# uber-research/UPSNet

Hardware: NVIDIA H100
Metric: panoptic images/sec at 1024x2048 (higher is better)
Workload: dtype bf16x3

## Files before the change

### upsnet_b200/build.py

```python
import os
import shutil
import subprocess
import sys

HERE = os.path.dirname(os.path.abspath(__file__))
CSRC = os.path.join(HERE, "csrc")
LIB = os.path.join(HERE, "libupsnet_b200.so")
SOURCES = ["roi_align.cu", "nms.cu", "panoptic.cu", "igemm_simt.cu", "igemm_tc.cu", "igemm_tma.cu", "dcn_win.cu", "detection.cu", "pool.cu", "post.cu", "impost.cu", "pq.cu", "sseg.cu", "cocoeval.cu", "combined.cu", "rpn_target.cu", "proposal_target.cu", "panoptic_loss.cu", "train_loss.cu", "labels.cu", "backward.cu", "conv_backward.cu", "sgd.cu", "capi.cu"]
NVCC_FLAGS = ["-gencode", "arch=compute_90a,code=sm_90a", "-O3", "-lineinfo", "-std=c++17",
              "-Xcompiler", "-fPIC", "--expt-relaxed-constexpr"]


def nvcc():
    for home in (os.environ.get("CUDA_HOME"), os.environ.get("CUDA_PATH")):
        if home and os.path.exists(os.path.join(home, "bin", "nvcc")):
            return os.path.join(home, "bin", "nvcc")
    return shutil.which("nvcc") or "/usr/local/cuda/bin/nvcc"


def _stale():
    if not os.path.exists(LIB):
        return True
    t = os.path.getmtime(LIB)
    deps = [os.path.join(CSRC, f) for f in os.listdir(CSRC)]
    deps.append(os.path.join(HERE, "..", "include", "upsnet_b200.h"))
    return any(os.path.getmtime(d) > t for d in deps)


def build(force=False, verbose=False):
    if not force and not _stale():
        return LIB
    objs = []
    procs = []
    os.makedirs(os.path.join(HERE, "build"), exist_ok=True)
    for src in SOURCES:
        obj = os.path.join(HERE, "build", src.replace(".cu", ".o"))
        cmd = [nvcc()] + NVCC_FLAGS + (["-Xptxas", "-v"] if verbose else []) + \
              ["-c", os.path.join(CSRC, src), "-o", obj]
        procs.append((src, subprocess.Popen(cmd, stdout=subprocess.PIPE, stderr=subprocess.STDOUT, text=True)))
        objs.append(obj)
    failed = False
    for src, pr in procs:
        out, _ = pr.communicate()
        if pr.returncode != 0 or verbose:
            sys.stderr.write("== %s ==\n%s\n" % (src, out))
        failed |= pr.returncode != 0
    if failed:
        raise RuntimeError("nvcc failed")
    subprocess.check_call([nvcc()] + NVCC_FLAGS[:2] + ["-shared", "-o", LIB] + objs + ["-lcudart"])
    return LIB


if __name__ == "__main__":
    print(build(force="--force" in sys.argv, verbose="-v" in sys.argv))
```

### upsnet_b200/csrc/igemm_tc.cu

```cuda
#include <cuda_bf16.h>
#include <cstdio>

#include "common.cuh"
#include "tc_ptx.cuh"
#include "tc_params.cuh"

namespace ups {

constexpr int TC_BM = 128;
constexpr int TC_BK = 64;
constexpr int TC_GROUP = 256;
constexpr int TC_GROUPS = 2;
constexpr int TC_PRODUCERS = TC_GROUP * TC_GROUPS;
constexpr int TC_CONSUMERS = 128;
constexpr int TC_EPI_PITCH = 36;
constexpr int TC_THREADS = TC_CONSUMERS + TC_PRODUCERS;
constexpr int TC_MAX_STAGES = 6;



struct TcSmem {
  uint32_t bars;
  uint32_t rowbase;
  uint32_t epi;
// ... 527 lines not shown
            size_t ridx = oidx;
            if (p.res_up2) {
              const int ho = pp / p.Wo, wo = pp - ho * p.Wo;
              ridx = (((size_t)n_img * (p.Ho >> 1) + (ho >> 1)) * (p.Wo >> 1) + (wo >> 1)) * p.Cout + co0;
            }
            const bool full = (co0 + 15 < p.Cout) && ((p.Cout & 7) == 0) && vec_ptrs_ok;
            if (p.y_bf16) {
              __nv_bfloat16* yo = reinterpret_cast<__nv_bfloat16*>(p.y) + oidx;
              const __nv_bfloat16* ro = p.residual ? reinterpret_cast<const __nv_bfloat16*>(p.residual) + ridx : nullptr;
              if (full) {
                if (ro) {
                  const uint4 r0 = __ldg(reinterpret_cast<const uint4*>(ro)), r1 = __ldg(reinterpret_cast<const uint4*>(ro) + 1);
                  const uint32_t rw[8] = {r0.x, r0.y, r0.z, r0.w, r1.x, r1.y, r1.z, r1.w};
#pragma unroll
                  for (int q = 0; q < 8; ++q) {
                    o16[2 * q] += bf16x2_x(rw[q]);
                    o16[2 * q + 1] += bf16x2_y(rw[q]);
                  }
                }
                if (p.relu) {
#pragma unroll
                  for (int e = 0; e < 16; ++e) o16[e] = fmaxf(o16[e], 0.f);
                }
                reinterpret_cast<uint4*>(yo)[0] = pack_bf16x8(o16);
                reinterpret_cast<uint4*>(yo)[1] = pack_bf16x8(o16 + 8);
              } else {
#pragma unroll
                for (int e = 0; e < 16; ++e) {
                  if (co0 + e >= p.Cout) break;
                  float o = o16[e];
                  if (ro) o += __bfloat162float(ro[e]);
                  if (p.relu) o = fmaxf(o, 0.f);
                  yo[e] = __float2bfloat16_rn(o);
                }
              }
            } else {
              float* yo = reinterpret_cast<float*>(p.y) + oidx;
              const float* ro = p.residual ? reinterpret_cast<const float*>(p.residual) + ridx : nullptr;
              if (full) {
#pragma unroll
                for (int g4 = 0; g4 < 4; ++g4) {
                  float4 o = make_float4(o16[g4 * 4], o16[g4 * 4 + 1], o16[g4 * 4 + 2], o16[g4 * 4 + 3]);
                  if (ro) {
                    const float4 rv = __ldg(reinterpret_cast<const float4*>(ro + g4 * 4));
                    o.x += rv.x; o.y += rv.y; o.z += rv.z; o.w += rv.w;
                  }
                  if (p.relu) { o.x = fmaxf(o.x, 0.f); o.y = fmaxf(o.y, 0.f); o.z = fmaxf(o.z, 0.f); o.w = fmaxf(o.w, 0.f); }
                  *reinterpret_cast<float4*>(yo + g4 * 4) = o;
                }
              } else {
#pragma unroll
                for (int e = 0; e < 16; ++e) {
                  if (co0 + e >= p.Cout) break;
                  float o = o16[e];
                  if (ro) o += __ldg(ro + e);
                  if (p.relu) o = fmaxf(o, 0.f);
                  yo[e] = o;
                }
              }
            }
          } else {
#pragma unroll
            for (int e = 0; e < 16; ++e) {
              const int co = co0 + e;
              if (co >= p.Cout) break;
              const size_t oidx = ((size_t)n_img * p.Cout + co) * HoWo + pp;
              float o = o16[e];
              if (p.y_bf16) {
                if (p.residual) o += __bfloat162float(reinterpret_cast<const __nv_bfloat16*>(p.residual)[oidx]);
                if (p.relu) o = fmaxf(o, 0.f);
                reinterpret_cast<__nv_bfloat16*>(p.y)[oidx] = __float2bfloat16_rn(o);
              } else {
                if (p.residual) o += __ldg(reinterpret_cast<const float*>(p.residual) + oidx);
                if (p.relu) o = fmaxf(o, 0.f);
                if (p.sig_from >= 0 && co >= p.sig_from) o = 1.f / (1.f + expf(-o));
                reinterpret_cast<float*>(p.y)[oidx] = o;
              }
            }
          }
        }
      }
    }
  }
}

__global__ void pack_weight_kernel(const float* __restrict__ w, int Cout, int Cin, int KHW, int Cout_pad, int Kp,
                                   uint16_t* __restrict__ hi, uint16_t* __restrict__ lo) {
  const size_t total = (size_t)Cout_pad * Kp;
  for (size_t i = (size_t)blockIdx.x * blockDim.x + threadIdx.x; i < total; i += (size_t)gridDim.x * blockDim.x) {
    const int kk = (int)(i % (size_t)Kp);
    const int co = (int)(i / (size_t)Kp);
    const int tap = kk / Cin, c = kk - tap * Cin;
    const float v = (co < Cout && kk < KHW * Cin) ? w[((size_t)co * Cin + c) * KHW + tap] : 0.f;
    __nv_bfloat16 h, l;
    split_bf16(v, h, l);
    hi[i] = *reinterpret_cast<const uint16_t*>(&h);
    lo[i] = *reinterpret_cast<const uint16_t*>(&l);
  }
}

static int tc_kp(int Cin, int KHW) { return (KHW * Cin + TC_BK - 1) / TC_BK * TC_BK; }

size_t tc_packed_weight_bytes(int Cout, int Cin, int kh, int kw) {
  return (size_t)2 * cout_pad(Cout) * tc_kp(Cin, kh * kw) * sizeof(uint16_t);
}

int tc_pack_weight(const float* w, int Cout, int Cin, int kh, int kw, void* packed, cudaStream_t stream) {
  const int Cout_pad = cout_pad(Cout), KHW = kh * kw, Kp = tc_kp(Cin, KHW);
  uint16_t* hi = reinterpret_cast<uint16_t*>(packed);
  uint16_t* lo = hi + (size_t)Cout_pad * Kp;
  const size_t total = (size_t)Cout_pad * Kp;
  int blocks = (int)((total + 255) / 256);
  if (blocks > kNumSMs * 16) blocks = kNumSMs * 16;
  pack_weight_kernel<<<blocks, 256, 0, stream>>>(w, Cout, Cin, KHW, Cout_pad, Kp, hi, lo);
  UPS_CHECK_LAUNCH();
  return 0;
}

bool tc_supported(int Cin, int kh, int kw, int dg) {
  return ((Cin % TC_BK) == 0 || Cin <= 8) && dg == 1 && kh * kw <= 49 && kh <= 15 && kw <= 15;
}

template <int BN>
static cudaError_t tc_configure() {
  const void* k[] = {(const void*)igemm_tc_kernel<0, 0, BN>, (const void*)igemm_tc_kernel<0, 1, BN>, (const void*)igemm_tc_kernel<0, 2, BN>,
                     (const void*)igemm_tc_kernel<1, 0, BN>, (const void*)igemm_tc_kernel<1, 1, BN>, (const void*)igemm_tc_kernel<1, 2, BN>,
                     (const void*)igemm_tc_kernel<2, 0, BN>};
  for (const void* f : k) {
    const cudaError_t e = cudaFuncSetAttribute(f, cudaFuncAttributeMaxDynamicSharedMemorySize, 227 * 1024);
    if (e != cudaSuccess) return e;
  }
  for (int i = 3; i < 6; ++i) (void)cudaFuncSetAttribute(k[i], cudaFuncAttributePreferredSharedMemoryCarveout, 60);
  return cudaSuccess;
}

template <int BN>
static void tc_launch(const TcParams& p, bool deform, bool smallc, dim3 grid, size_t smem, cudaStream_t stream) {
  if (smallc) igemm_tc_kernel<2, 0, BN><<<grid, TC_THREADS, smem, stream>>>(p);
  else if (p.x_pair) {
    if (deform) igemm_tc_kernel<1, 2, BN><<<grid, TC_THREADS, smem, stream>>>(p);
    else igemm_tc_kernel<0, 2, BN><<<grid, TC_THREADS, smem, stream>>>(p);
  } else if (p.x_bf16) {
    if (deform) igemm_tc_kernel<1, 1, BN><<<grid, TC_THREADS, smem, stream>>>(p);
    else igemm_tc_kernel<0, 1, BN><<<grid, TC_THREADS, smem, stream>>>(p);
  } else {
    if (deform) igemm_tc_kernel<1, 0, BN><<<grid, TC_THREADS, smem, stream>>>(p);
    else igemm_tc_kernel<0, 0, BN><<<grid, TC_THREADS, smem, stream>>>(p);
  }
}

int launch_igemm_tc(TcParams p, const void* packed, cudaStream_t stream) {
  const int KHW = p.kh * p.kw;
  if (!tc_supported(p.Cin, p.kh, p.kw, 1)) return UPSNET_E_UNSUPPORTED;
  {
    const int rc = launch_igemm_tma(p, packed, stream);
    if (rc != UPSNET_E_UNSUPPORTED) return rc;
  }
  if ((((uintptr_t)p.x) & 15) || (((uintptr_t)packed) & 15) || (((uintptr_t)p.y) & 15)) return UPSNET_E_BADARG;
  p.Cout_pad = cout_pad(p.Cout);
  p.w_hi = reinterpret_cast<const uint16_t*>(packed);
  p.w_lo = p.w_hi + (size_t)p.Cout_pad * tc_kp(p.Cin, KHW);
  const bool deform = p.offset != nullptr;
  const bool smallc = (p.Cin % TC_BK) != 0;
  if (deform && (p.x_bf16 || p.x_pair) && (long long)p.H * p.W * p.Cin * (p.x_pair ? 2 : 1) >= (1ll << 31)) return UPSNET_E_UNSUPPORTED;
  if (smallc && (deform || p.x_bf16 || p.x_pair || p.dh * (p.kh - 1) > 255 || p.dw * (p.kw - 1) > 255)) return UPSNET_E_UNSUPPORTED;
  if (p.x_pair && !p.x3) return UPSNET_E_UNSUPPORTED;
  if (p.sig_from >= 0 && (p.out_nhwc || p.y_bf16)) return UPSNET_E_UNSUPPORTED;
  if (p.x_bf16 && !p.x_pair && p.x3) return UPSNET_E_UNSUPPORTED;
  if (p.y_pair) {
    if (!p.out_nhwc || (p.Cout & 7) || (p.pair_group && p.pair_group != p.Cout)) return UPSNET_E_UNSUPPORTED;
    if (p.residual && (((uintptr_t)p.residual) & 15)) return UPSNET_E_UNSUPPORTED;
  }
  int BN = p.Cout_pad > 64 ? 64 : p.Cout_pad;
  {
    const long long mt = ((long long)p.N * p.Ho * p.Wo + TC_BM - 1) / TC_BM;
    while (BN > 64 && (BN % 32) == 0 && mt * (p.Cout_pad / BN) < kNumSMs && p.Cout_pad % (BN / 2) == 0 && ((BN / 2) % 32) == 0) BN /= 2;
  }
  p.BN = BN;
  const int khw_l = smallc ? 2 : KHW;
  int stages = deform ? 3 : TC_MAX_STAGES;
  TcSmem L = tc_smem_layout(deform, khw_l, BN, stages, p.x3 != 0);
  while (stages > 2 && L.total + 1024 > 220 * 1024) { --stages; L = tc_smem_layout(deform, khw_l, BN, stages, p.x3 != 0); }
  if (L.total + 1024 > 227 * 1024) return UPSNET_E_UNSUPPORTED;
  p.stages = stages;
  const long long Ptot = (long long)p.N * p.Ho * p.Wo;
  if (Ptot <= 0) return 0;
  const int sms = num_sms();
  p.tile_w = 16; p.tile_h = 8;
  auto dtiles = [&]() { return (long long)p.N * ((p.Wo + p.tile_w - 1) / p.tile_w) * ((p.Ho + p.tile_h - 1) / p.tile_h) * (p.Cout_pad / BN); };
  if (deform) {
    if (dtiles() < sms / 2) { p.tile_w = 8; p.tile_h = 8; }
    if (dtiles() < sms / 2) { p.tile_h = 4; }
  }
  const long long num_tiles = (deform ? dtiles() : ((Ptot + TC_BM - 1) / TC_BM) * (p.Cout_pad / BN));
  dim3 grid((unsigned)(num_tiles < sms ? num_tiles : sms));
  const size_t smem = L.total + 1024;
  static PerDeviceOnce configured;
  if (configured.need()) {
    UPS_CUDA(tc_configure<32>());
    UPS_CUDA(tc_configure<64>());
  }
  switch (BN) {
    case 32: tc_launch<32>(p, deform, smallc, grid, smem, stream); break;
    case 64: tc_launch<64>(p, deform, smallc, grid, smem, stream); break;
    default: return UPSNET_E_UNSUPPORTED;
  }
  UPS_CHECK_LAUNCH();
  return 0;
}

}
```

### upsnet_b200/csrc/tc_params.cuh

```cuda
#pragma once
#include <cuda.h>
#include <cuda_runtime.h>
#include <cstdint>

namespace ups {

inline int cout_pad(int Cout) { return Cout <= 32 ? 32 : (Cout + 63) / 64 * 64; }

typedef CUresult (*EncodeTiledFn)(CUtensorMap*, CUtensorMapDataType, cuuint32_t, void*, const cuuint64_t*, const cuuint64_t*,
                                  const cuuint32_t*, const cuuint32_t*, CUtensorMapInterleave, CUtensorMapSwizzle,
                                  CUtensorMapL2promotion, CUtensorMapFloatOOBfill);

inline EncodeTiledFn tma_encoder() {
  static EncodeTiledFn fn = nullptr;
  static bool tried = false;
  if (!tried) {
    void* p = nullptr;
    cudaDriverEntryPointQueryResult qr = cudaDriverEntryPointSymbolNotFound;
    if (cudaGetDriverEntryPoint("cuTensorMapEncodeTiled", &p, cudaEnableDefault, &qr) == cudaSuccess &&
        qr == cudaDriverEntryPointSuccess)
      fn = reinterpret_cast<EncodeTiledFn>(p);
    else
      (void)cudaGetLastError();
    tried = true;
  }
  return fn;
}

struct TcParams {
  const void* x;
  const float* offset;
  const float* mask;
  const uint16_t* w_hi;
  const uint16_t* w_lo;
  const float* bias; const void* residual; void* y;
  int N, H, W, Cin, Cout, Cout_pad, kh, kw, sh, sw, ph, pw, dh, dw, Ho, Wo;
  int relu, out_nhwc, BN, stages, x3;
  int x_bf16, y_bf16;
  int x_pair, y_pair;
  int sig_from;
  int pair_group;
  int res_up2;
  int no_tma;
  int tile_w, tile_h;
  const int* n_dev;
};

size_t tc_packed_weight_bytes(int Cout, int Cin, int kh, int kw);
int tc_pack_weight(const float* w, int Cout, int Cin, int kh, int kw, void* packed, cudaStream_t stream);
bool tc_supported(int Cin, int kh, int kw, int dg);
int launch_igemm_tc(TcParams p, const void* packed, cudaStream_t stream);
int launch_igemm_tma(const TcParams& p, const void* packed, cudaStream_t stream);

}
```

### upsnet_b200/csrc/tc_ptx.cuh

```cuda
#pragma once
#include <cuda.h>
#include <cuda_bf16.h>
#include <cstdint>
#include <cstdio>

#include "pair.cuh"

namespace ups {

__device__ __forceinline__ uint32_t smem_u32(const void* p) { return (uint32_t)__cvta_generic_to_shared(p); }

__device__ __forceinline__ void mbar_init(uint32_t bar, uint32_t count) {
  asm volatile("mbarrier.init.shared::cta.b64 [%0], %1;" ::"r"(bar), "r"(count));
}
__device__ __forceinline__ void mbar_arrive(uint32_t bar) {
  asm volatile("mbarrier.arrive.shared::cta.b64 _, [%0];" ::"r"(bar) : "memory");
}
__device__ __forceinline__ bool mbar_try_wait(uint32_t bar, uint32_t parity) {
  uint32_t ok;
  asm volatile(
      "{\n\t.reg .pred p;\n\t"
      "mbarrier.try_wait.parity.shared::cta.b64 p, [%1], %2;\n\t"
      "selp.u32 %0, 1, 0, p;\n\t}"
      : "=r"(ok) : "r"(bar), "r"(parity) : "memory");
  return ok != 0;
}
__device__ __forceinline__ void mbar_wait(uint32_t bar, uint32_t parity) {
  uint32_t spins = 0;
  long long t0 = 0;
  while (!mbar_try_wait(bar, parity)) {
    if ((++spins & 1023u) == 0) {
      const long long now = clock64();
      if (t0 == 0) t0 = now;
      else if (now - t0 > 4000000000LL) __trap();
    }
  }
}
__device__ __forceinline__ void fence_mbar_init() { asm volatile("fence.mbarrier_init.release.cluster;" ::: "memory"); }
__device__ __forceinline__ void fence_proxy_async() { asm volatile("fence.proxy.async.shared::cta;" ::: "memory"); }

__device__ __forceinline__ void mbar_arrive_expect_tx(uint32_t bar, uint32_t bytes) {
  asm volatile("mbarrier.arrive.expect_tx.shared::cta.b64 _, [%0], %1;" ::"r"(bar), "r"(bytes) : "memory");
}
__device__ __forceinline__ void tma_load_2d(uint32_t dst, const CUtensorMap* tm, uint32_t bar, int c0, int c1) {
  asm volatile(
      "cp.async.bulk.tensor.2d.shared::cluster.global.tile.mbarrier::complete_tx::bytes [%0], [%1, {%3, %4}], [%2];"
      ::"r"(dst), "l"(reinterpret_cast<uint64_t>(tm)), "r"(bar), "r"(c0), "r"(c1) : "memory");
}
__device__ __forceinline__ void tma_load_4d(uint32_t dst, const CUtensorMap* tm, uint32_t bar, int c0, int c1, int c2, int c3) {
  asm volatile(
      "cp.async.bulk.tensor.4d.shared::cluster.global.tile.mbarrier::complete_tx::bytes [%0], [%1, {%3, %4, %5, %6}], [%2];"
      ::"r"(dst), "l"(reinterpret_cast<uint64_t>(tm)), "r"(bar), "r"(c0), "r"(c1), "r"(c2), "r"(c3) : "memory");
}
__device__ __forceinline__ void tma_load_5d(uint32_t dst, const CUtensorMap* tm, uint32_t bar, int c0, int c1, int c2, int c3, int c4) {
  asm volatile(
      "cp.async.bulk.tensor.5d.shared::cluster.global.tile.mbarrier::complete_tx::bytes [%0], [%1, {%3, %4, %5, %6, %7}], [%2];"
      ::"r"(dst), "l"(reinterpret_cast<uint64_t>(tm)), "r"(bar), "r"(c0), "r"(c1), "r"(c2), "r"(c3), "r"(c4) : "memory");
}
__device__ __forceinline__ void tma_store_4d(const CUtensorMap* tm, uint32_t src, int c0, int c1, int c2, int c3) {
  asm volatile(
      "cp.async.bulk.tensor.4d.global.shared::cta.tile.bulk_group [%0, {%2, %3, %4, %5}], [%1];"
      ::"l"(reinterpret_cast<uint64_t>(tm)), "r"(src), "r"(c0), "r"(c1), "r"(c2), "r"(c3) : "memory");
}
__device__ __forceinline__ void bulk_commit() { asm volatile("cp.async.bulk.commit_group;" ::: "memory"); }
__device__ __forceinline__ void bulk_wait_read0() { asm volatile("cp.async.bulk.wait_group.read 0;" ::: "memory"); }
__device__ __forceinline__ void bulk_wait_read1() { asm volatile("cp.async.bulk.wait_group.read 1;" ::: "memory"); }
__device__ __forceinline__ void bulk_wait0() { asm volatile("cp.async.bulk.wait_group 0;" ::: "memory"); }
__device__ __forceinline__ void prefetch_tmap(const CUtensorMap* tm) {
  asm volatile("prefetch.tensormap [%0];" ::"l"(reinterpret_cast<uint64_t>(tm)) : "memory");
}

template <int R> __device__ __forceinline__ void setmaxnreg_inc() { asm volatile("setmaxnreg.inc.sync.aligned.u32 %0;" ::"n"(R)); }
template <int R> __device__ __forceinline__ void setmaxnreg_dec() { asm volatile("setmaxnreg.dec.sync.aligned.u32 %0;" ::"n"(R)); }

template <int N> struct Wgmma;
template <> struct Wgmma<32> {
  static __device__ __forceinline__ void mma(float (&d)[16], uint64_t da, uint64_t db, uint32_t accumulate) {
    asm volatile(
        "{\n\t.reg .pred p;\n\tsetp.ne.b32 p, %18, 0;\n\t"
        "wgmma.mma_async.sync.aligned.m64n32k16.f32.bf16.bf16 {%0, %1, %2, %3, %4, %5, %6, %7, %8, %9, %10, %11, %12, %13, %14, %15}, %16, %17, p, 1, 1, 0, 0;\n\t}"
        : "+f"(d[0]), "+f"(d[1]), "+f"(d[2]), "+f"(d[3]), "+f"(d[4]), "+f"(d[5]), "+f"(d[6]), "+f"(d[7]), "+f"(d[8]), "+f"(d[9]), "+f"(d[10]), "+f"(d[11]), "+f"(d[12]), "+f"(d[13]), "+f"(d[14]), "+f"(d[15])
        : "l"(da), "l"(db), "r"(accumulate));
  }
};
template <> struct Wgmma<64> {
  static __device__ __forceinline__ void mma(float (&d)[32], uint64_t da, uint64_t db, uint32_t accumulate) {
    asm volatile(
        "{\n\t.reg .pred p;\n\tsetp.ne.b32 p, %34, 0;\n\t"
        "wgmma.mma_async.sync.aligned.m64n64k16.f32.bf16.bf16 {%0, %1, %2, %3, %4, %5, %6, %7, %8, %9, %10, %11, %12, %13, %14, %15, %16, %17, %18, %19, %20, %21, %22, %23, %24, %25, %26, %27, %28, %29, %30, %31}, %32, %33, p, 1, 1, 0, 0;\n\t}"
        : "+f"(d[0]), "+f"(d[1]), "+f"(d[2]), "+f"(d[3]), "+f"(d[4]), "+f"(d[5]), "+f"(d[6]), "+f"(d[7]), "+f"(d[8]), "+f"(d[9]), "+f"(d[10]), "+f"(d[11]), "+f"(d[12]), "+f"(d[13]), "+f"(d[14]), "+f"(d[15]), "+f"(d[16]), "+f"(d[17]), "+f"(d[18]), "+f"(d[19]), "+f"(d[20]), "+f"(d[21]), "+f"(d[22]), "+f"(d[23]), "+f"(d[24]), "+f"(d[25]), "+f"(d[26]), "+f"(d[27]), "+f"(d[28]), "+f"(d[29]), "+f"(d[30]), "+f"(d[31])
        : "l"(da), "l"(db), "r"(accumulate));
  }
};
template <> struct Wgmma<96> {
  static __device__ __forceinline__ void mma(float (&d)[48], uint64_t da, uint64_t db, uint32_t accumulate) {
    asm volatile(
        "{\n\t.reg .pred p;\n\tsetp.ne.b32 p, %50, 0;\n\t"
        "wgmma.mma_async.sync.aligned.m64n96k16.f32.bf16.bf16 {%0, %1, %2, %3, %4, %5, %6, %7, %8, %9, %10, %11, %12, %13, %14, %15, %16, %17, %18, %19, %20, %21, %22, %23, %24, %25, %26, %27, %28, %29, %30, %31, %32, %33, %34, %35, %36, %37, %38, %39, %40, %41, %42, %43, %44, %45, %46, %47}, %48, %49, p, 1, 1, 0, 0;\n\t}"
        : "+f"(d[0]), "+f"(d[1]), "+f"(d[2]), "+f"(d[3]), "+f"(d[4]), "+f"(d[5]), "+f"(d[6]), "+f"(d[7]), "+f"(d[8]), "+f"(d[9]), "+f"(d[10]), "+f"(d[11]), "+f"(d[12]), "+f"(d[13]), "+f"(d[14]), "+f"(d[15]), "+f"(d[16]), "+f"(d[17]), "+f"(d[18]), "+f"(d[19]), "+f"(d[20]), "+f"(d[21]), "+f"(d[22]), "+f"(d[23]), "+f"(d[24]), "+f"(d[25]), "+f"(d[26]), "+f"(d[27]), "+f"(d[28]), "+f"(d[29]), "+f"(d[30]), "+f"(d[31]), "+f"(d[32]), "+f"(d[33]), "+f"(d[34]), "+f"(d[35]), "+f"(d[36]), "+f"(d[37]), "+f"(d[38]), "+f"(d[39]), "+f"(d[40]), "+f"(d[41]), "+f"(d[42]), "+f"(d[43]), "+f"(d[44]), "+f"(d[45]), "+f"(d[46]), "+f"(d[47])
        : "l"(da), "l"(db), "r"(accumulate));
  }
};
template <> struct Wgmma<128> {
  static __device__ __forceinline__ void mma(float (&d)[64], uint64_t da, uint64_t db, uint32_t accumulate) {
    asm volatile(
        "{\n\t.reg .pred p;\n\tsetp.ne.b32 p, %66, 0;\n\t"
        "wgmma.mma_async.sync.aligned.m64n128k16.f32.bf16.bf16 {%0, %1, %2, %3, %4, %5, %6, %7, %8, %9, %10, %11, %12, %13, %14, %15, %16, %17, %18, %19, %20, %21, %22, %23, %24, %25, %26, %27, %28, %29, %30, %31, %32, %33, %34, %35, %36, %37, %38, %39, %40, %41, %42, %43, %44, %45, %46, %47, %48, %49, %50, %51, %52, %53, %54, %55, %56, %57, %58, %59, %60, %61, %62, %63}, %64, %65, p, 1, 1, 0, 0;\n\t}"
        : "+f"(d[0]), "+f"(d[1]), "+f"(d[2]), "+f"(d[3]), "+f"(d[4]), "+f"(d[5]), "+f"(d[6]), "+f"(d[7]), "+f"(d[8]), "+f"(d[9]), "+f"(d[10]), "+f"(d[11]), "+f"(d[12]), "+f"(d[13]), "+f"(d[14]), "+f"(d[15]), "+f"(d[16]), "+f"(d[17]), "+f"(d[18]), "+f"(d[19]), "+f"(d[20]), "+f"(d[21]), "+f"(d[22]), "+f"(d[23]), "+f"(d[24]), "+f"(d[25]), "+f"(d[26]), "+f"(d[27]), "+f"(d[28]), "+f"(d[29]), "+f"(d[30]), "+f"(d[31]), "+f"(d[32]), "+f"(d[33]), "+f"(d[34]), "+f"(d[35]), "+f"(d[36]), "+f"(d[37]), "+f"(d[38]), "+f"(d[39]), "+f"(d[40]), "+f"(d[41]), "+f"(d[42]), "+f"(d[43]), "+f"(d[44]), "+f"(d[45]), "+f"(d[46]), "+f"(d[47]), "+f"(d[48]), "+f"(d[49]), "+f"(d[50]), "+f"(d[51]), "+f"(d[52]), "+f"(d[53]), "+f"(d[54]), "+f"(d[55]), "+f"(d[56]), "+f"(d[57]), "+f"(d[58]), "+f"(d[59]), "+f"(d[60]), "+f"(d[61]), "+f"(d[62]), "+f"(d[63])
        : "l"(da), "l"(db), "r"(accumulate));
  }
};
template <> struct Wgmma<256> {
  static __device__ __forceinline__ void mma(float (&d)[128], uint64_t da, uint64_t db, uint32_t accumulate) {
    asm volatile(
        "{\n\t.reg .pred p;\n\tsetp.ne.b32 p, %130, 0;\n\t"
        "wgmma.mma_async.sync.aligned.m64n256k16.f32.bf16.bf16 {%0, %1, %2, %3, %4, %5, %6, %7, %8, %9, %10, %11, %12, %13, %14, %15, %16, %17, %18, %19, %20, %21, %22, %23, %24, %25, %26, %27, %28, %29, %30, %31, %32, %33, %34, %35, %36, %37, %38, %39, %40, %41, %42, %43, %44, %45, %46, %47, %48, %49, %50, %51, %52, %53, %54, %55, %56, %57, %58, %59, %60, %61, %62, %63, %64, %65, %66, %67, %68, %69, %70, %71, %72, %73, %74, %75, %76, %77, %78, %79, %80, %81, %82, %83, %84, %85, %86, %87, %88, %89, %90, %91, %92, %93, %94, %95, %96, %97, %98, %99, %100, %101, %102, %103, %104, %105, %106, %107, %108, %109, %110, %111, %112, %113, %114, %115, %116, %117, %118, %119, %120, %121, %122, %123, %124, %125, %126, %127}, %128, %129, p, 1, 1, 0, 0;\n\t}"
        : "+f"(d[0]), "+f"(d[1]), "+f"(d[2]), "+f"(d[3]), "+f"(d[4]), "+f"(d[5]), "+f"(d[6]), "+f"(d[7]), "+f"(d[8]), "+f"(d[9]), "+f"(d[10]), "+f"(d[11]), "+f"(d[12]), "+f"(d[13]), "+f"(d[14]), "+f"(d[15]), "+f"(d[16]), "+f"(d[17]), "+f"(d[18]), "+f"(d[19]), "+f"(d[20]), "+f"(d[21]), "+f"(d[22]), "+f"(d[23]), "+f"(d[24]), "+f"(d[25]), "+f"(d[26]), "+f"(d[27]), "+f"(d[28]), "+f"(d[29]), "+f"(d[30]), "+f"(d[31]), "+f"(d[32]), "+f"(d[33]), "+f"(d[34]), "+f"(d[35]), "+f"(d[36]), "+f"(d[37]), "+f"(d[38]), "+f"(d[39]), "+f"(d[40]), "+f"(d[41]), "+f"(d[42]), "+f"(d[43]), "+f"(d[44]), "+f"(d[45]), "+f"(d[46]), "+f"(d[47]), "+f"(d[48]), "+f"(d[49]), "+f"(d[50]), "+f"(d[51]), "+f"(d[52]), "+f"(d[53]), "+f"(d[54]), "+f"(d[55]), "+f"(d[56]), "+f"(d[57]), "+f"(d[58]), "+f"(d[59]), "+f"(d[60]), "+f"(d[61]), "+f"(d[62]), "+f"(d[63]), "+f"(d[64]), "+f"(d[65]), "+f"(d[66]), "+f"(d[67]), "+f"(d[68]), "+f"(d[69]), "+f"(d[70]), "+f"(d[71]), "+f"(d[72]), "+f"(d[73]), "+f"(d[74]), "+f"(d[75]), "+f"(d[76]), "+f"(d[77]), "+f"(d[78]), "+f"(d[79]), "+f"(d[80]), "+f"(d[81]), "+f"(d[82]), "+f"(d[83]), "+f"(d[84]), "+f"(d[85]), "+f"(d[86]), "+f"(d[87]), "+f"(d[88]), "+f"(d[89]), "+f"(d[90]), "+f"(d[91]), "+f"(d[92]), "+f"(d[93]), "+f"(d[94]), "+f"(d[95]), "+f"(d[96]), "+f"(d[97]), "+f"(d[98]), "+f"(d[99]), "+f"(d[100]), "+f"(d[101]), "+f"(d[102]), "+f"(d[103]), "+f"(d[104]), "+f"(d[105]), "+f"(d[106]), "+f"(d[107]), "+f"(d[108]), "+f"(d[109]), "+f"(d[110]), "+f"(d[111]), "+f"(d[112]), "+f"(d[113]), "+f"(d[114]), "+f"(d[115]), "+f"(d[116]), "+f"(d[117]), "+f"(d[118]), "+f"(d[119]), "+f"(d[120]), "+f"(d[121]), "+f"(d[122]), "+f"(d[123]), "+f"(d[124]), "+f"(d[125]), "+f"(d[126]), "+f"(d[127])
        : "l"(da), "l"(db), "r"(accumulate));
  }
};

template <int N> struct WgmmaT;
template <> struct WgmmaT<128> {
  static __device__ __forceinline__ void mma(float (&d)[64], uint64_t da, uint64_t db, uint32_t accumulate) {
    asm volatile(
        "{\n\t.reg .pred p;\n\tsetp.ne.b32 p, %66, 0;\n\t"
        "wgmma.mma_async.sync.aligned.m64n128k16.f32.bf16.bf16 {%0, %1, %2, %3, %4, %5, %6, %7, %8, %9, %10, %11, %12, %13, %14, %15, %16, %17, %18, %19, %20, %21, %22, %23, %24, %25, %26, %27, %28, %29, %30, %31, %32, %33, %34, %35, %36, %37, %38, %39, %40, %41, %42, %43, %44, %45, %46, %47, %48, %49, %50, %51, %52, %53, %54, %55, %56, %57, %58, %59, %60, %61, %62, %63}, %64, %65, p, 1, 1, 1, 1;\n\t}"
        : "+f"(d[0]), "+f"(d[1]), "+f"(d[2]), "+f"(d[3]), "+f"(d[4]), "+f"(d[5]), "+f"(d[6]), "+f"(d[7]), "+f"(d[8]), "+f"(d[9]), "+f"(d[10]), "+f"(d[11]), "+f"(d[12]), "+f"(d[13]), "+f"(d[14]), "+f"(d[15]), "+f"(d[16]), "+f"(d[17]), "+f"(d[18]), "+f"(d[19]), "+f"(d[20]), "+f"(d[21]), "+f"(d[22]), "+f"(d[23]), "+f"(d[24]), "+f"(d[25]), "+f"(d[26]), "+f"(d[27]), "+f"(d[28]), "+f"(d[29]), "+f"(d[30]), "+f"(d[31]), "+f"(d[32]), "+f"(d[33]), "+f"(d[34]), "+f"(d[35]), "+f"(d[36]), "+f"(d[37]), "+f"(d[38]), "+f"(d[39]), "+f"(d[40]), "+f"(d[41]), "+f"(d[42]), "+f"(d[43]), "+f"(d[44]), "+f"(d[45]), "+f"(d[46]), "+f"(d[47]), "+f"(d[48]), "+f"(d[49]), "+f"(d[50]), "+f"(d[51]), "+f"(d[52]), "+f"(d[53]), "+f"(d[54]), "+f"(d[55]), "+f"(d[56]), "+f"(d[57]), "+f"(d[58]), "+f"(d[59]), "+f"(d[60]), "+f"(d[61]), "+f"(d[62]), "+f"(d[63])
        : "l"(da), "l"(db), "r"(accumulate));
  }
};

__device__ __forceinline__ void wgmma_fence() { asm volatile("wgmma.fence.sync.aligned;" ::: "memory"); }
__device__ __forceinline__ void wgmma_commit() { asm volatile("wgmma.commit_group.sync.aligned;" ::: "memory"); }
template <int PENDING> __device__ __forceinline__ void wgmma_wait() {
  asm volatile("wgmma.wait_group.sync.aligned %0;" ::"n"(PENDING) : "memory");
}
template <int R> __device__ __forceinline__ void wgmma_fence_acc(float (&d)[R]) {
#pragma unroll
  for (int i = 0; i < R; ++i) asm volatile("" : "+f"(d[i])::"memory");
}

__device__ __forceinline__ uint32_t wg_desc_lo(uint32_t smem_addr) { return ((smem_addr >> 4) & 0x3fffu) | (1u << 16); }
__device__ __forceinline__ uint32_t wg_desc_hi(uint32_t sbo_bytes) { return (sbo_bytes >> 4) | (1u << 30); }
__device__ __forceinline__ uint32_t wg_desc_hi_sw64(uint32_t sbo_bytes) { return (sbo_bytes >> 4) | (2u << 30); }
__device__ __forceinline__ uint64_t wg_desc(uint32_t lo, uint32_t hi) { return ((uint64_t)hi << 32) | lo; }
__device__ __forceinline__ uint32_t wg_desc_mn_lo(uint32_t smem_addr, uint32_t lbo_bytes) {
  return ((smem_addr >> 4) & 0x3fffu) | ((lbo_bytes >> 4) << 16);
}

template <int N, int NC>
__device__ __forceinline__ void acc_stage(const float (&d)[N / 2], float* buf, int pitch, int row0, int c0) {
  const int t = threadIdx.x & 127, l = t & 31;
  const int r = row0 + 16 * (t >> 5) + (l >> 2);
#pragma unroll
  for (int i = 0; i < N / 8; ++i) {
    if (8 * i < c0 || 8 * i >= c0 + NC) continue;
    const int c = 8 * i - c0 + 2 * (l & 3);
    *reinterpret_cast<float2*>(buf + (size_t)r * pitch + c) = make_float2(d[4 * i], d[4 * i + 1]);
    *reinterpret_cast<float2*>(buf + (size_t)(r + 8) * pitch + c) = make_float2(d[4 * i + 2], d[4 * i + 3]);
  }
}
__device__ __forceinline__ void acc_ld16(uint32_t addr, uint32_t (&r)[16]) {
#pragma unroll
  for (int i = 0; i < 4; ++i)
    asm volatile("ld.shared.v4.b32 {%0, %1, %2, %3}, [%4];"
                 : "=r"(r[4 * i]), "=r"(r[4 * i + 1]), "=r"(r[4 * i + 2]), "=r"(r[4 * i + 3]) : "r"(addr + 16u * i));
}
__device__ __forceinline__ uint4 lds128(uint32_t addr) {
  uint4 v;
  asm volatile("ld.shared.v4.u32 {%0, %1, %2, %3}, [%4];" : "=r"(v.x), "=r"(v.y), "=r"(v.z), "=r"(v.w) : "r"(addr));
  return v;
}
__device__ __forceinline__ void sts128(uint32_t addr, const uint4& v) {
  asm volatile("st.shared.v4.u32 [%0], {%1, %2, %3, %4};" ::"r"(addr), "r"(v.x), "r"(v.y), "r"(v.z), "r"(v.w) : "memory");
}
__device__ __forceinline__ uint32_t lds32(uint32_t addr) {
  uint32_t v;
  asm volatile("ld.shared.b32 %0, [%1];" : "=r"(v) : "r"(addr));
  return v;
}
__device__ __forceinline__ void sts32(uint32_t addr, uint32_t v) {
  asm volatile("st.shared.b32 [%0], %1;" ::"r"(addr), "r"(v) : "memory");
}
__device__ __forceinline__ void named_bar(int id, int count) { asm volatile("bar.sync %0, %1;" ::"r"(id), "r"(count) : "memory"); }
template <int ID, int COUNT> __device__ __forceinline__ void named_bar() { asm volatile("bar.sync %0, %1;" ::"n"(ID), "n"(COUNT) : "memory"); }

__device__ __forceinline__ void cp_async16(uint32_t dst_smem, const void* src) {
  asm volatile("cp.async.cg.shared.global [%0], [%1], 16;" ::"r"(dst_smem), "l"(src) : "memory");
}
__device__ __forceinline__ void cp_async16_zfill(uint32_t dst_smem, const void* src, uint32_t src_bytes) {
  asm volatile("cp.async.cg.shared.global [%0], [%1], 16, %2;" ::"r"(dst_smem), "l"(src), "r"(src_bytes) : "memory");
}
__device__ __forceinline__ void cp_async_commit() { asm volatile("cp.async.commit_group;" ::: "memory"); }
__device__ __forceinline__ void cp_async_wait_all() { asm volatile("cp.async.wait_group 0;" ::: "memory"); }
__device__ __forceinline__ void cp_async_wait_but2() { asm volatile("cp.async.wait_group 2;" ::: "memory"); }

__device__ __forceinline__ void ldg256(const void* p, uint4& lo, uint4& hi) {
  lo = __ldg(reinterpret_cast<const uint4*>(p));
  hi = __ldg(reinterpret_cast<const uint4*>(p) + 1);
// ... 13 lines not shown
```

Before: 129.4.

## Add specialized thin-output 3x3 conv kernel using TMA and mma.sync bf16x3

Adds a dedicated persistent kernel for 3x3 stride-1 convolutions with few output channels (Cout<=32, a multiple of 9, e.g. the RPN/mask heads) over paired-bf16 inputs. It loads halo tiles and weights via TMA into a double-buffered ring and computes with mma.sync in a three-product hi/lo split. A host-side cost model chooses the row blocking and optional K-split. It targets the waste the generic igemm kernels incur by padding tiny Cout to 32/64, at the cost of extra code paths and an uncoalesced NCHW fp32 store.

```diff
diff --git a/upsnet_b200/build.py b/upsnet_b200/build.py
--- a/upsnet_b200/build.py
+++ b/upsnet_b200/build.py
@@ -6,7 +6,7 @@
 HERE = os.path.dirname(os.path.abspath(__file__))
 CSRC = os.path.join(HERE, "csrc")
 LIB = os.path.join(HERE, "libupsnet_b200.so")
-SOURCES = ["roi_align.cu", "nms.cu", "panoptic.cu", "igemm_simt.cu", "igemm_tc.cu", "igemm_tma.cu", "dcn_win.cu", "detection.cu", "pool.cu", "post.cu", "impost.cu", "pq.cu", "sseg.cu", "cocoeval.cu", "combined.cu", "rpn_target.cu", "proposal_target.cu", "panoptic_loss.cu", "train_loss.cu", "labels.cu", "backward.cu", "conv_backward.cu", "sgd.cu", "capi.cu"]
+SOURCES = ["roi_align.cu", "nms.cu", "panoptic.cu", "igemm_simt.cu", "igemm_tc.cu", "igemm_tma.cu", "conv_thin.cu", "dcn_win.cu", "detection.cu", "pool.cu", "post.cu", "impost.cu", "pq.cu", "sseg.cu", "cocoeval.cu", "combined.cu", "rpn_target.cu", "proposal_target.cu", "panoptic_loss.cu", "train_loss.cu", "labels.cu", "backward.cu", "conv_backward.cu", "sgd.cu", "capi.cu"]
 NVCC_FLAGS = ["-gencode", "arch=compute_90a,code=sm_90a", "-O3", "-lineinfo", "-std=c++17",
               "-Xcompiler", "-fPIC", "--expt-relaxed-constexpr"]
 
diff --git a/upsnet_b200/csrc/conv_thin.cu b/upsnet_b200/csrc/conv_thin.cu
--- /dev/null
+++ b/upsnet_b200/csrc/conv_thin.cu
@@ -0,0 +1,283 @@
+#include <cuda.h>
+#include <cuda_bf16.h>
+#include <cuda_runtime.h>
+#include <cstdint>
+
+#include "common.cuh"
+#include "tc_params.cuh"
+#include "tc_ptx.cuh"
+
+namespace ups {
+
+constexpr int CT_THREADS = 256;
+constexpr int CT_BW = 32;
+constexpr int CT_HW = CT_BW + 2;
+constexpr int CT_CH = 32;
+constexpr int CT_STAGES = 2;
+
+struct ThinGeom {
+  const float* bias;
+  float* y;
+  int N, Ho, Wo, Cin, Cout;
+  int w_lo;
+  int tiles_w, tiles_h;
+};
+
+__host__ __device__ constexpr int ct_bh(int R, int KS) { return R * 4 / KS; }
+
+__host__ __device__ constexpr uint32_t ct_align(uint32_t v) { return (v + 1023u) & ~1023u; }
+__host__ __device__ constexpr uint32_t ct_x_bytes(int BH) { return (uint32_t)(BH + 2) * CT_HW * CT_CH * 2; }
+__host__ __device__ constexpr uint32_t ct_w_bytes(int NT) { return (uint32_t)(8 * NT) * 9 * CT_CH * 2; }
+__host__ __device__ constexpr uint32_t ct_stage_bytes(int BH, int NT) { return 2 * ct_align(ct_x_bytes(BH)) + 2 * ct_align(ct_w_bytes(NT)); }
+__host__ __device__ constexpr uint32_t ct_red_bytes(int R, int NT, int KS) { return KS > 1 ? 4u * 32u * R * NT * 16u : 0u; }
+__host__ __device__ constexpr uint32_t ct_smem_bytes(int R, int NT, int KS) {
+  return 1024 + 1024 + CT_STAGES * ct_stage_bytes(ct_bh(R, KS), NT) + ct_red_bytes(R, NT, KS);
+}
+
+__device__ __forceinline__ uint32_t sw64(uint32_t r, uint32_t c) { return r * 64u + ((c ^ ((r >> 1) & 3u)) << 4); }
+
+__device__ __forceinline__ void ldsm_x4(uint32_t addr, uint32_t (&r)[4]) {
+  asm volatile("ldmatrix.sync.aligned.m8n8.x4.shared.b16 {%0, %1, %2, %3}, [%4];"
+               : "=r"(r[0]), "=r"(r[1]), "=r"(r[2]), "=r"(r[3]) : "r"(addr));
+}
+__device__ __forceinline__ void ldsm_x2(uint32_t addr, uint32_t (&r)[2]) {
+  asm volatile("ldmatrix.sync.aligned.m8n8.x2.shared.b16 {%0, %1}, [%2];" : "=r"(r[0]), "=r"(r[1]) : "r"(addr));
+}
+__device__ __forceinline__ void mma_bf16(float (&d)[4], const uint32_t (&a)[4], uint32_t b0, uint32_t b1) {
+  asm("mma.sync.aligned.m16n8k16.row.col.f32.bf16.bf16.f32 {%0, %1, %2, %3}, {%4, %5, %6, %7}, {%8, %9}, {%0, %1, %2, %3};"
+      : "+f"(d[0]), "+f"(d[1]), "+f"(d[2]), "+f"(d[3])
+      : "r"(a[0]), "r"(a[1]), "r"(a[2]), "r"(a[3]), "r"(b0), "r"(b1));
+}
+
+template <int R, int NT, int KS>
+__global__ void __launch_bounds__(CT_THREADS, R == 1 ? 2 : 1)
+conv_thin3x3_kernel(const __grid_constant__ CUtensorMap tm_x, const __grid_constant__ CUtensorMap tm_w, const ThinGeom g) {
+  constexpr int BH = ct_bh(R, KS), WG = 8 / KS;
+  constexpr uint32_t XB = ct_align(ct_x_bytes(BH)), WB = ct_align(ct_w_bytes(NT)), SB = ct_stage_bytes(BH, NT);
+  extern __shared__ __align__(1024) uint8_t smem_dyn[];
+  const uint32_t raw = smem_u32(smem_dyn);
+  const uint32_t base = (raw + 1023u) & ~1023u;
+  const uint32_t bar = base;
+  const uint32_t ring = base + 1024;
+  float4* red = reinterpret_cast<float4*>(smem_dyn + (base - raw) + 1024 + CT_STAGES * SB);
+
+  const int tid = threadIdx.x, warp = tid >> 5, lane = tid & 31;
+  const int kg = warp / WG, mw = warp % WG;
+  const int col0 = (mw & 1) * 16, row0 = (mw >> 1) * R;
+  const int nch = g.Cin / CT_CH;
+  const long long tiles = (long long)g.N * g.tiles_h * g.tiles_w;
+  const long long my_tiles = tiles > blockIdx.x ? (tiles - 1 - blockIdx.x) / gridDim.x + 1 : 0;
+  const long long iters = my_tiles * nch;
+
+  auto tile_origin = [&](long long j, int& n, int& y0, int& x0) {
+    const long long t = blockIdx.x + j * gridDim.x;
+    x0 = (int)(t % g.tiles_w) * CT_BW;
+    y0 = (int)((t / g.tiles_w) % g.tiles_h) * BH;
+    n = (int)(t / ((long long)g.tiles_w * g.tiles_h));
+  };
+  auto load = [&](long long i) {
+    const int s = (int)(i % CT_STAGES), c = (int)(i % nch);
+    int n, y0, x0;
+    tile_origin(i / nch, n, y0, x0);
+    const uint32_t st = ring + (uint32_t)s * SB, b = bar + 8u * (uint32_t)s;
+    mbar_arrive_expect_tx(b, 2u * ct_x_bytes(BH) + 2u * ct_w_bytes(NT));
+    tma_load_4d(st, &tm_x, b, c * CT_CH, x0 - 1, y0 - 1, n);
+    tma_load_4d(st + XB, &tm_x, b, g.Cin + c * CT_CH, x0 - 1, y0 - 1, n);
+    tma_load_3d(st + 2 * XB, &tm_w, b, c * CT_CH, 0, 0);
+    tma_load_3d(st + 2 * XB + WB, &tm_w, b, c * CT_CH, 0, g.w_lo);
+  };
+
+  if (tid == 0) {
+    prefetch_tmap(&tm_x);
+    prefetch_tmap(&tm_w);
+    for (int s = 0; s < CT_STAGES; ++s) mbar_init(bar + 8u * s, 1);
+    fence_mbar_init();
+    for (long long i = 0; i < CT_STAGES && i < iters; ++i) load(i);
+  }
+  __syncthreads();
+
+  const uint32_t a_pix = (uint32_t)(row0 * CT_HW + col0 + (lane & 15));
+  const uint32_t a_half = (uint32_t)(lane >> 4), b_half = (uint32_t)((lane >> 3) & 1), b_n = (uint32_t)(lane & 7);
+
+  float acc[R][NT][4];
+#pragma unroll
+  for (int r = 0; r < R; ++r)
+#pragma unroll
+    for (int t = 0; t < NT; ++t)
+#pragma unroll
+      for (int e = 0; e < 4; ++e) acc[r][t][e] = 0.f;
+
+  for (long long i = 0; i < iters; ++i) {
+    const int s = (int)(i % CT_STAGES), c = (int)(i % nch);
+    mbar_wait(bar + 8u * (uint32_t)s, (uint32_t)((i / CT_STAGES) & 1));
+    const uint32_t xh = ring + (uint32_t)s * SB, xl = xh + XB, wh = xh + 2 * XB, wl = wh + WB;
+#pragma unroll
+    for (int kk = 0; kk < 2 / KS; ++kk) {
+      const uint32_t k = KS == 1 ? (uint32_t)kk : (uint32_t)kg;
+#pragma unroll
+      for (int kx = 0; kx < 3; ++kx) {
+        uint32_t ahi[R + 2][4], alo[R + 2][4];
+#pragma unroll
+        for (int h = 0; h < R + 2; ++h) {
+          const uint32_t q = a_pix + (uint32_t)(h * CT_HW + kx);
+          ldsm_x4(xh + sw64(q, 2 * k + a_half), ahi[h]);
+          ldsm_x4(xl + sw64(q, 2 * k + a_half), alo[h]);
+        }
+#pragma unroll
+        for (int ky = 0; ky < 3; ++ky) {
+          uint32_t bhi[NT][2], blo[NT][2];
+#pragma unroll
+          for (int t = 0; t < NT; ++t) {
+            const uint32_t q = (uint32_t)(t * 8 + b_n) * 9u + (uint32_t)(ky * 3 + kx);
+            ldsm_x2(wh + sw64(q, 2 * k + b_half), bhi[t]);
+            ldsm_x2(wl + sw64(q, 2 * k + b_half), blo[t]);
+          }
+#pragma unroll
+          for (int r = 0; r < R; ++r) {
+#pragma unroll
+            for (int t = 0; t < NT; ++t) mma_bf16(acc[r][t], ahi[r + ky], bhi[t][0], bhi[t][1]);
+#pragma unroll
+            for (int t = 0; t < NT; ++t) mma_bf16(acc[r][t], ahi[r + ky], blo[t][0], blo[t][1]);
+#pragma unroll
+            for (int t = 0; t < NT; ++t) mma_bf16(acc[r][t], alo[r + ky], bhi[t][0], bhi[t][1]);
+          }
+        }
+      }
+    }
+    __syncthreads();
+    if (tid == 0 && i + CT_STAGES < iters) load(i + CT_STAGES);
+
+    if (c == nch - 1) {
+      if constexpr (KS == 2) {
+        if (kg == 1) {
+#pragma unroll
+          for (int r = 0; r < R; ++r)
+#pragma unroll
+            for (int t = 0; t < NT; ++t) {
+              red[((r * NT + t) * WG + mw) * 32 + lane] = make_float4(acc[r][t][0], acc[r][t][1], acc[r][t][2], acc[r][t][3]);
+              acc[r][t][0] = acc[r][t][1] = acc[r][t][2] = acc[r][t][3] = 0.f;
+            }
+        }
+        __syncthreads();
+        if (kg == 1) continue;
+#pragma unroll
+        for (int r = 0; r < R; ++r)
+#pragma unroll
+          for (int t = 0; t < NT; ++t) {
+            const float4 v = red[((r * NT + t) * WG + mw) * 32 + lane];
+            acc[r][t][0] += v.x; acc[r][t][1] += v.y; acc[r][t][2] += v.z; acc[r][t][3] += v.w;
+          }
+      }
+      int n, y0, x0;
+      tile_origin(i / nch, n, y0, x0);
+      const size_t plane = (size_t)g.Ho * g.Wo;
+#pragma unroll
+      for (int r = 0; r < R; ++r) {
+        const int oy = y0 + row0 + r;
+#pragma unroll
+        for (int t = 0; t < NT; ++t) {
+#pragma unroll
+          for (int e = 0; e < 4; ++e) {
+            const int ox = x0 + col0 + (lane >> 2) + 8 * (e >> 1);
+            const int co = t * 8 + 2 * (lane & 3) + (e & 1);
+            if (oy < g.Ho && ox < g.Wo && co < g.Cout) {
+              float o = acc[r][t][e];
+              if (g.bias) o += __ldg(g.bias + co);
+              g.y[((size_t)n * g.Cout + co) * plane + (size_t)oy * g.Wo + ox] = o;
+            }
+            acc[r][t][e] = 0.f;
+          }
+        }
+      }
+    }
+  }
+}
+
+static int ct_per_sm(uint32_t smem) { return smem <= 113u * 1024u ? 2 : 1; }
+
+template <int R, int NT, int KS>
+static int ct_launch(const CUtensorMap& tm_x, const CUtensorMap& tm_w, const ThinGeom& g, long long tiles, cudaStream_t stream) {
+  const int sms = num_sms();
+  const uint32_t smem = ct_smem_bytes(R, NT, KS);
+  const long long cap = (long long)sms * ct_per_sm(smem);
+  const dim3 grid((unsigned)(tiles < cap ? tiles : cap));
+  conv_thin3x3_kernel<R, NT, KS><<<grid, CT_THREADS, smem, stream>>>(tm_x, tm_w, g);
+  UPS_CHECK_LAUNCH();
+  return 0;
+}
+
+template <int R, int NT, int KS>
+static cudaError_t ct_opt_in() {
+  return cudaFuncSetAttribute((const void*)conv_thin3x3_kernel<R, NT, KS>, cudaFuncAttributeMaxDynamicSharedMemorySize,
+                              (int)ct_smem_bytes(R, NT, KS));
+}
+
+bool conv_thin_applies(const TcParams& p) {
+  return p.x_pair && p.x3 && !p.no_tma && !p.offset && !p.n_dev && p.kh == 3 && p.kw == 3 && p.sh == 1 && p.sw == 1 &&
+         p.ph == 1 && p.pw == 1 && p.dh == 1 && p.dw == 1 && p.Cout <= 32 && (p.Cout % 9) == 0 && (p.Cin % 64) == 0 && !p.out_nhwc &&
+         !p.y_bf16 && !p.y_pair && !p.relu && !p.residual && !p.res_up2 && p.sig_from < 0;
+}
+
+int launch_conv_thin(const TcParams& p, const void* packed, cudaStream_t stream) {
+  if ((((uintptr_t)p.x) & 15) || (((uintptr_t)packed) & 15)) return UPSNET_E_BADARG;
+  EncodeTiledFn enc = tma_encoder();
+  if (!enc) return UPSNET_E_UNSUPPORTED;
+  const int NT = (p.Cout + 7) / 8;
+  const int tiles_w = (p.Wo + CT_BW - 1) / CT_BW;
+  auto tiles_of = [&](int bh) { return (long long)p.N * tiles_w * ((p.Ho + bh - 1) / bh); };
+  const int cand[3][3] = {{4, 1, 8}, {2, 1, 9}, {1, 2, 12}};
+  int R = 0, KS = 0;
+  long long best = -1;
+  for (const auto& rk : cand) {
+    if (rk[0] == 4 && NT > 3) continue;
+    const int bh = ct_bh(rk[0], rk[1]), per = ct_per_sm(ct_smem_bytes(rk[0], NT, rk[1]));
+    const long long cap = (long long)num_sms() * per;
+    const long long cost = (tiles_of(bh) + cap - 1) / cap * per * bh * rk[2];
+    if (best < 0 || cost < best) { best = cost; R = rk[0]; KS = rk[1]; }
+  }
+  const int BH = ct_bh(R, KS);
+  ThinGeom g{};
+  g.bias = p.bias; g.y = reinterpret_cast<float*>(p.y);
+  g.N = p.N; g.Ho = p.Ho; g.Wo = p.Wo; g.Cin = p.Cin; g.Cout = p.Cout; g.w_lo = cout_pad(p.Cout);
+  g.tiles_w = tiles_w; g.tiles_h = (p.Ho + BH - 1) / BH;
+  const long long tiles = tiles_of(BH);
+
+  CUtensorMap tm_x, tm_w;
+  const cuuint32_t es[4] = {1, 1, 1, 1};
+  {
+    const cuuint64_t dims[4] = {(cuuint64_t)2 * p.Cin, (cuuint64_t)p.W, (cuuint64_t)p.H, (cuuint64_t)p.N};
+    const cuuint64_t strides[3] = {(cuuint64_t)p.Cin * 4, (cuuint64_t)p.W * p.Cin * 4, (cuuint64_t)p.H * p.W * p.Cin * 4};
+    const cuuint32_t box[4] = {CT_CH, CT_HW, (cuuint32_t)BH + 2, 1};
+    if (enc(&tm_x, CU_TENSOR_MAP_DATA_TYPE_BFLOAT16, 4, const_cast<void*>(p.x), dims, strides, box, es, CU_TENSOR_MAP_INTERLEAVE_NONE,
+            CU_TENSOR_MAP_SWIZZLE_64B, CU_TENSOR_MAP_L2_PROMOTION_L2_128B, CU_TENSOR_MAP_FLOAT_OOB_FILL_NONE) != CUDA_SUCCESS)
+      return UPSNET_E_UNSUPPORTED;
+  }
+  {
+    const cuuint64_t dims[3] = {(cuuint64_t)p.Cin, 9, (cuuint64_t)2 * g.w_lo};
+    const cuuint64_t strides[2] = {(cuuint64_t)p.Cin * 2, (cuuint64_t)9 * p.Cin * 2};
+    const cuuint32_t box[3] = {CT_CH, 9, (cuuint32_t)(8 * NT)};
+    if (enc(&tm_w, CU_TENSOR_MAP_DATA_TYPE_BFLOAT16, 3, const_cast<void*>(packed), dims, strides, box, es, CU_TENSOR_MAP_INTERLEAVE_NONE,
+            CU_TENSOR_MAP_SWIZZLE_64B, CU_TENSOR_MAP_L2_PROMOTION_L2_128B, CU_TENSOR_MAP_FLOAT_OOB_FILL_NONE) != CUDA_SUCCESS)
+      return UPSNET_E_UNSUPPORTED;
+  }
+  if (tiles <= 0) return 0;
+  static PerDeviceOnce configured;
+  if (configured.need()) {
+    UPS_CUDA((ct_opt_in<4, 2, 1>())); UPS_CUDA((ct_opt_in<4, 3, 1>()));
+    UPS_CUDA((ct_opt_in<2, 2, 1>())); UPS_CUDA((ct_opt_in<2, 3, 1>())); UPS_CUDA((ct_opt_in<2, 4, 1>()));
+    UPS_CUDA((ct_opt_in<1, 2, 2>())); UPS_CUDA((ct_opt_in<1, 3, 2>())); UPS_CUDA((ct_opt_in<1, 4, 2>()));
+  }
+  switch (R * 100 + KS * 10 + NT) {
+    case 412: return ct_launch<4, 2, 1>(tm_x, tm_w, g, tiles, stream);
+    case 413: return ct_launch<4, 3, 1>(tm_x, tm_w, g, tiles, stream);
+    case 212: return ct_launch<2, 2, 1>(tm_x, tm_w, g, tiles, stream);
+    case 213: return ct_launch<2, 3, 1>(tm_x, tm_w, g, tiles, stream);
+    case 214: return ct_launch<2, 4, 1>(tm_x, tm_w, g, tiles, stream);
+    case 122: return ct_launch<1, 2, 2>(tm_x, tm_w, g, tiles, stream);
+    case 123: return ct_launch<1, 3, 2>(tm_x, tm_w, g, tiles, stream);
+    case 124: return ct_launch<1, 4, 2>(tm_x, tm_w, g, tiles, stream);
+    default: return UPSNET_E_UNSUPPORTED;
+  }
+}
+
+}
diff --git a/upsnet_b200/csrc/igemm_tc.cu b/upsnet_b200/csrc/igemm_tc.cu
--- a/upsnet_b200/csrc/igemm_tc.cu
+++ b/upsnet_b200/csrc/igemm_tc.cu
@@ -703,6 +703,10 @@
 int launch_igemm_tc(TcParams p, const void* packed, cudaStream_t stream) {
   const int KHW = p.kh * p.kw;
   if (!tc_supported(p.Cin, p.kh, p.kw, 1)) return UPSNET_E_UNSUPPORTED;
+  if (conv_thin_applies(p)) {
+    const int rc = launch_conv_thin(p, packed, stream);
+    if (rc != UPSNET_E_UNSUPPORTED) return rc;
+  }
   {
     const int rc = launch_igemm_tma(p, packed, stream);
     if (rc != UPSNET_E_UNSUPPORTED) return rc;
diff --git a/upsnet_b200/csrc/tc_params.cuh b/upsnet_b200/csrc/tc_params.cuh
--- a/upsnet_b200/csrc/tc_params.cuh
+++ b/upsnet_b200/csrc/tc_params.cuh
@@ -51,5 +51,7 @@
 bool tc_supported(int Cin, int kh, int kw, int dg);
 int launch_igemm_tc(TcParams p, const void* packed, cudaStream_t stream);
 int launch_igemm_tma(const TcParams& p, const void* packed, cudaStream_t stream);
+bool conv_thin_applies(const TcParams& p);
+int launch_conv_thin(const TcParams& p, const void* packed, cudaStream_t stream);
 
 }
diff --git a/upsnet_b200/csrc/tc_ptx.cuh b/upsnet_b200/csrc/tc_ptx.cuh
--- a/upsnet_b200/csrc/tc_ptx.cuh
+++ b/upsnet_b200/csrc/tc_ptx.cuh
@@ -46,6 +46,11 @@
   asm volatile(
       "cp.async.bulk.tensor.2d.shared::cluster.global.tile.mbarrier::complete_tx::bytes [%0], [%1, {%3, %4}], [%2];"
       ::"r"(dst), "l"(reinterpret_cast<uint64_t>(tm)), "r"(bar), "r"(c0), "r"(c1) : "memory");
+}
+__device__ __forceinline__ void tma_load_3d(uint32_t dst, const CUtensorMap* tm, uint32_t bar, int c0, int c1, int c2) {
+  asm volatile(
+      "cp.async.bulk.tensor.3d.shared::cluster.global.tile.mbarrier::complete_tx::bytes [%0], [%1, {%3, %4, %5}], [%2];"
+      ::"r"(dst), "l"(reinterpret_cast<uint64_t>(tm)), "r"(bar), "r"(c0), "r"(c1), "r"(c2) : "memory");
 }
 __device__ __forceinline__ void tma_load_4d(uint32_t dst, const CUtensorMap* tm, uint32_t bar, int c0, int c1, int c2, int c3) {
   asm volatile(
```

After: 132.1, median of 6. 1.02x the previous value.
